# roahmlab/koopman-realizations

Hardware: AMD Instinct MI355X
Metric: EDMD snapshot-pairs/sec (bilinear fit, 3-link arm, poly-3) (higher is better)
Workload: dtype f64

## Files before the change

### koopman-realizations_amd/csrc/kp_context.hip

```cpp
#include <algorithm>
#include <cmath>
#include <cstring>
#include <mutex>

#include "kp_internal.h"

static std::mutex g_err_mu;
static std::string g_err;

void kp_set_global_error(const std::string& s) {
  std::lock_guard<std::mutex> l(g_err_mu);
  g_err = s;
}

void* kp_ctx::workspace(int slot, size_t bytes) {
  if (ws_bytes[slot] >= bytes && ws[slot]) return ws[slot];
  if (ws[slot]) (void)hipFree(ws[slot]);
  ws[slot] = nullptr;
  ws_bytes[slot] = 0;
  size_t want = bytes + bytes / 4 + 256;
  if (hipMalloc(&ws[slot], want) != hipSuccess) return nullptr;
  ws_bytes[slot] = want;
  return ws[slot];
}
// ... 94 lines not shown
  copy = g_err;
  return copy.c_str();
}

extern "C" int kp_device_info(const kp_ctx* c, char* name, int name_len, int* num_cu, int64_t* hbm) {
  if (!c) return KP_ERR_ARG;
  if (name && name_len > 0) {
    std::strncpy(name, c->name.c_str(), (size_t)name_len - 1);
    name[name_len - 1] = 0;
  }
  if (num_cu) *num_cu = c->num_cu;
  if (hbm) *hbm = c->hbm_bytes;
  return KP_OK;
}

void* kp_pinned_scratch(kp_ctx* ctx, size_t bytes) {
  if (ctx->pin_scratch_bytes >= bytes) return ctx->pin_scratch;
  if (ctx->pin_scratch) {
    (void)hipStreamSynchronize(ctx->stream);
    (void)hipHostFree(ctx->pin_scratch);
  }
  ctx->pin_scratch = nullptr;
  ctx->pin_scratch_bytes = 0;
  const size_t cap = (bytes + 4095) & ~(size_t)4095;
  if (hipHostMalloc(&ctx->pin_scratch, cap, hipHostMallocDefault) != hipSuccess) {
    ctx->pin_scratch = nullptr;
    return nullptr;
  }
  ctx->pin_scratch_bytes = cap;
  return ctx->pin_scratch;
}

extern "C" int kp_timer_get(const kp_ctx* c, int which, double* ms) {
  if (!c || !ms || which < 0 || which >= 20) return KP_ERR_ARG;
  *ms = c->timers[which];
  return KP_OK;
}

extern "C" void* kp_stream(const kp_ctx* c) { return c ? (void*)c->stream : nullptr; }


static int upload(kp_ctx* ctx, void** dst, const void* src, size_t bytes) {
  *dst = nullptr;
  if (bytes == 0) return KP_OK;
  KP_HIP(ctx, hipMalloc(dst, bytes));
  KP_HIP(ctx, hipMemcpy(*dst, src, bytes, hipMemcpyHostToDevice));
  return KP_OK;
}

extern "C" int kp_basis_desc_dims(const kp_basis_desc* d, int* nvars_out, int* nfull_out, int* N_out, int* W_out) {
  if (!d || d->nzeta < 1 || d->m < 0 || d->model_type < 0 || d->model_type > 2 || d->n_blocks < 0 ||
      (d->n_blocks && (!d->block_type || !d->block_count)))
    return KP_ERR_ARG;
  const int nvars = d->nzeta + (d->model_type == KP_MODEL_NONLINEAR ? d->m : 0);
  double nf = nvars + 1.0;
  for (int b = 0; b < d->n_blocks; ++b) {
    const int c = d->block_count[b];
    if (c < 0) return KP_ERR_ARG;
    switch (d->block_type[b]) {
      case KP_BLOCK_POLY: case KP_BLOCK_HERMITE: case KP_BLOCK_FOURIER_SPARSER: case KP_BLOCK_GAUSSIAN: nf += c; break;
      case KP_BLOCK_FOURIER: nf += std::pow((double)(2 * c + 1), (double)nvars) - 1.0; break;
      default: return KP_ERR_ARG;
    }
    if (nf > 1e6) return KP_ERR_ARG;
  }
  const int nfull = (int)std::llround(nf);
  const int N = d->k_pcs > 0 ? d->k_pcs + nvars + 1 : nfull;
// ... 430 lines not shown
```

### koopman-realizations_amd/csrc/kp_gram3.hip

```cpp
#include <algorithm>
#include <cstdlib>
#include <type_traits>
#include <vector>

#include "kp_internal.h"

#ifndef KP_RAW_STEP
#define KP_RAW_STEP 1
#endif
#define KT3 8
#define NF3 3
#define RS3 240
#define YOFF3 96
#define ZOFF3 192
#define WOFF3 196
#define SOFF3 208
#define NIDMAX3 144
#define PST3 10
#define POWBUF3 (PST3 * NIDMAX3)
#define PSIBUF3 (KT3 * RS3)
#define PSI03 (2 * POWBUF3)
#define LDS3_DOUBLES (PSI03 + 2 * PSIBUF3)
#define PCS03 LDS3_DOUBLES
#define PCSMAX3 32
#define LDS3_PCS_DOUBLES (2 * YOFF3 * 16)
#define GC03 LDS3_DOUBLES
#define GAUSSMAX3 32
#ifndef KP_PCS_REGS
#define KP_PCS_REGS 24
#endif
#define GNZMAX3 8
#define LDS3_GAUSS_DOUBLES (GAUSSMAX3 * GNZMAX3)

#include "kp_gram3_args.h"
#include "kp_gram3_cover.h"

__device__ double kp_gram3_ones[KT3] = {1.0, 1.0, 1.0, 1.0, 1.0, 1.0, 1.0, 1.0};

template <int NQ, int BM, bool PCS, bool EXT = false, bool PRE = false, bool TUP = false, bool P3 = false>
__global__ __launch_bounds__(256, 2) void kp_gram3_kernel(Gram3Args a) {
  constexpr int NWT = (BM + 1) * (BM + 2) / 2;
  static_assert(!P3 || (!PCS && !EXT && !PRE), "three-entry table: the in-kernel-lift monomial form");
  static_assert(!TUP || NWT % 2 == 0, "paired weights: an even number of weights (m = 3: 10 = 5 tuples, m = 2: 6 = 3 tuples)");
  auto wslot = [](int w) { return TUP ? 6 * (w & 1) + (w >> 1) : w - 1; };
  extern __shared__ __align__(16) double sm[];
  const BasisDev& b = a.b;
  const int tid = threadIdx.x;
  const int lane = tid & 63;
  const int wave = tid >> 6;
  const int per_xcd = gridDim.x / 8;
  const int logical = (int)blockIdx.x < per_xcd * 8 ? ((int)blockIdx.x % 8) * per_xcd + (int)blockIdx.x / 8 : (int)blockIdx.x;
  const int super = logical % a.nsuper;
  const int split = logical / a.nsuper;
  constexpr bool GRP = !PCS && !EXT && !PRE;
  const int fit = GRP ? __builtin_amdgcn_readfirstlane(split / a.nsplit_fit) : 0;
  const int split_local = split - fit * a.nsplit_fit;
  const double* const src_alpha = GRP ? a.grp[fit].alpha : a.alpha;
  const double* const src_beta = GRP ? a.grp[fit].beta : a.beta;
  const double* const src_u = GRP ? a.grp[fit].u : a.u;
  const int job = super * 4 + wave;
  const int nzm = b.nzeta + b.m;
  const int nrawrows = 2 * nzm;
  const int D = a.D;
  constexpr bool INL = !EXT && !PRE;
  const int RB = !INL ? D * PST3 : ((nrawrows + 1) * 62 + 4 * PST3 <= POWBUF3 ? 62 : 4 * PST3);
  const int CA = nrawrows * RB;

  const uint32_t* jd = a.desc + (size_t)job * (1 + NQ);
  const uint32_t jh = jd[0];
  const int lrow = (lane >> 4) * RS3, blk = (lane >> 2) & 3, lc = lane & 3;
  const int ao0 = PSI03 + lrow + 4 * (int)(jh & 255u) + lc;
  const int ao1 = PSI03 + lrow + 4 * (int)((jh >> 8) & 255u) + lc;
  const int qs = __builtin_amdgcn_readfirstlane((int)((jh >> 16) & 255u));
  int bo[NQ];
  int bo2[TUP ? NQ : 1];
// ... 15 lines not shown
    for (int w = 0; w < NWT; ++w) acc[q][w] = 0.0;

  auto item_setup = [&](int item, int (&fa_)[NF3], int& woff_) __attribute__((always_inline)) {
    const bool lvalid = item >= 0 && item < 2 * b.nfull;
    const int lside = (lvalid && item >= b.nfull) ? 1 : 0;
    const int lcol = lvalid ? item - lside * b.nfull : 0;
    const int lw = item - 2 * b.nfull;
    const bool lwt = lw >= 0 && lw < NWT - 1;
    const uint32_t r = lvalid ? a.recipes[lcol] : 0xffffffffu;
#pragma unroll
    for (int f = 0; f < NF3; ++f) {
      const int id = (int)((r >> (8 * f)) & 255u);
      fa_[f] = id == 255 ? CA : (EXT && id >= 128) ? CA + (1 + lside * a.ng + (id - 128)) * PST3 : (lside * nzm + id / D) * RB + (id % D) * PST3;
    }
    if (lwt) {
      int cnt = 0;
      for (int x = 0; x <= BM; ++x)
        for (int y = x; y <= BM; ++y) {
          if (cnt == lw + 1) {
            if (x > 0) fa_[0] = (b.nzeta + x - 1) * RB;
            if (y > 0) fa_[1] = (b.nzeta + y - 1) * RB;
          }
          ++cnt;
        }
    }
    woff_ = PSI03 + (lvalid ? lside * YOFF3 + lcol : lwt ? WOFF3 + wslot(lw + 1) : SOFF3 + (tid & 31));
  };
  constexpr int NLS = 3;
  int fs[NLS][NF3], ws[NLS];
  {
    const int nitems = 2 * b.nfull + NWT - 1;
#pragma unroll
    for (int j = 0; j < NLS; ++j) {
      const int e = tid + 256 * j;
      const bool on = e < 4 * nitems;
      const int ch = on ? e / nitems : 0;
      item_setup(on ? e - ch * nitems : -1, fs[j], ws[j]);
#pragma unroll
      for (int f = 0; f < NF3; ++f) fs[j][f] += 2 * ch;
      ws[j] += 2 * ch * RS3;
    }
  }

  const int64_t kt0 = (int64_t)split_local * a.ktiles_per_split;
  const int64_t ktiles_total = (a.Ns + KT3 - 1) / KT3;
  const int nkt = (int)max((int64_t)0, min((int64_t)a.ktiles_per_split, ktiles_total - kt0));

  constexpr int LR = 1;
  const int nld = (nrawrows * KT3 + 255) / 256;
  constexpr int LG = EXT ? 2 : 0;
  struct RawRegs { double v[LR]; bool ok; };
  bool ld_on[LR];
  bool ld_isz[LR];
  const double* ld_ptr[LR];
  const int ld_s = tid & (KT3 - 1);
  const int ld_dst0 = (tid / KT3) * RB + ld_s;
  int ld_rem = (int)max((int64_t)-1000000, min((int64_t)1 << 30, a.Ns - (kt0 * KT3 + ld_s)));
#pragma unroll
  for (int j = 0; j < LR; ++j) {
    const int e = tid + j * 256;
    ld_on[j] = e < nrawrows * KT3;
    const int r = ld_on[j] ? e / KT3 : 0;
    const int rr = r % nzm;
    const double* src = rr < b.nzeta ? ((r < nzm ? src_alpha : src_beta) + (int64_t)rr * a.Ns) : (src_u + (int64_t)(rr - b.nzeta) * a.Ns);
    ld_ptr[j] = src + kt0 * KT3 + ld_s;
    ld_isz[j] = ld_on[j] && rr < b.nzeta;
  }
  bool g_on[LG > 0 ? LG : 1];
  const double* g_ptr[LG > 0 ? LG : 1];
  int g_dst[LG > 0 ? LG : 1], g_cen[LG > 0 ? LG : 1];
  if (EXT) {
#pragma unroll
    for (int q = 0; q < LG; ++q) {
      const int gi = tid + q * 256;
      g_on[q] = gi < 2 * a.ng * KT3;
      const int gc = g_on[q] ? (gi / KT3) % a.ng : 0, gside = g_on[q] ? gi / (KT3 * a.ng) : 0;
// ... 123 lines not shown
  int pre_dst[2] = {0, 0};
  if (PRE) {
#pragma unroll
    for (int j = 0; j < 2; ++j) {
      const int e = tid + j * 256;
      pre_on[j] = e < pre_n2;
      const int e1 = pre_on[j] ? e : 0;
      const int sp = e1 / a.pre_rl, c = e1 - sp * a.pre_rl, srow = 2 * sp;
      const int cw = c - 8 * a.G4;
      const int off = c < 4 * a.G4 ? c : c < 8 * a.G4 ? YOFF3 + (c - 4 * a.G4) : WOFF3 + (!TUP ? cw : cw < NWT - 1 ? wslot(cw + 1) : (cw - (NWT - 1)) < 2 * (6 - NWT / 2) ? ((cw - (NWT - 1)) / (6 - NWT / 2)) * 6 + NWT / 2 + (cw - (NWT - 1)) % (6 - NWT / 2) : 12);
      pre_dst[j] = PSI03 + srow * RS3 + off;
    }
  }
  auto load_pre = [&]() __attribute__((always_inline)) -> PreRegs {
    PreRegs x;
    x.v[0] = make_double2(0.0, 0.0);
    x.v[1] = make_double2(0.0, 0.0);
    if (pre_left > 0) {
      if (pre_on[0]) x.v[0] = pre_ptr[0];
      if (pre_on[1]) x.v[1] = pre_ptr[256];
      pre_ptr += pre_n2;
    }
    --pre_left;
    return x;
  };
  auto store_pre = [&](auto buf_c, const PreRegs& x) __attribute__((always_inline)) {
    constexpr int BUF = decltype(buf_c)::value;
    if (pre_on[0]) { sm[BUF * PSIBUF3 + pre_dst[0]] = x.v[0].x; sm[BUF * PSIBUF3 + pre_dst[0] + RS3] = x.v[0].y; }
    if (pre_on[1]) { sm[BUF * PSIBUF3 + pre_dst[1]] = x.v[1].x; sm[BUF * PSIBUF3 + pre_dst[1] + RS3] = x.v[1].y; }
  };

  constexpr int NCH = NLS;
  double2 lf[NF3];
  auto lift_read = [&](int j, auto buf_c) __attribute__((always_inline)) {
    constexpr int BUF = decltype(buf_c)::value;
#pragma unroll
    for (int f = 0; f < NF3; ++f)
      lf[f] = *reinterpret_cast<const double2*>(__builtin_assume_aligned(&sm[BUF * POWBUF3 + fs[j][f]], 16));
  };
  auto lift_write = [&](int j, auto buf_c) __attribute__((always_inline)) {
    constexpr int BUF = decltype(buf_c)::value;
    sm[BUF * PSIBUF3 + ws[j]] = (lf[0].x * lf[1].x) * lf[2].x;
    sm[BUF * PSIBUF3 + ws[j] + RS3] = (lf[0].y * lf[1].y) * lf[2].y;
  };
  constexpr int WAIT_LGKM0 = 0xc07f;
  static_assert(WAIT_LGKM0 == ((63 & 15) | (7 << 4) | (0 << 8) | ((63 >> 4) << 14)), "vmcnt = 63 and expcnt = 7 (no wait), lgkmcnt = 0");
  auto lds_store_barrier = [&]() __attribute__((always_inline)) {
    __builtin_amdgcn_s_waitcnt(WAIT_LGKM0);
    __syncthreads();
  };
  using B0 = std::integral_constant<int, 0>;
  using B1 = std::integral_constant<int, 1>;

  constexpr int PREG = PCS ? KP_PCS_REGS : 1;
  double pcs_r[PREG];
  if (PCS) {
    __syncthreads();
    const int bbase0 = PCS03 + (lane >> 4) * 16 + 4 * blk + lc;
#pragma unroll
    for (int kk = 0; kk < PREG; ++kk) pcs_r[kk] = kk < a.nfull4 / 4 ? sm[bbase0 + kk * 64] : 0.0;
  }
  auto project = [&](auto buf_c) __attribute__((always_inline)) {
    constexpr int BUF = decltype(buf_c)::value;
    const int side = wave >> 1, rg = wave & 1;
    const int abase = BUF * PSIBUF3 + PSI03 + (4 * rg + lc) * RS3 + side * YOFF3 + (lane >> 4);
    const int bbase = PCS03 + (lane >> 4) * 16 + 4 * blk + lc;
    const int nf4 = a.nfull4;
    double p0 = 0.0, p1 = 0.0;
    const int bb1 = bbase + nf4 * 16;
    const int nk = nf4 / 4;
#pragma unroll
    for (int kk = 0; kk < PREG; ++kk) {
      if (kk < nk) {
        const double av = sm[abase + 4 * kk];
        const double b1 = sm[bb1 + kk * 64];
        p0 = __builtin_amdgcn_mfma_f64_4x4x4f64(av, pcs_r[kk], p0, 0, 0, 0);
// ... 15 lines not shown
      const int pc = 4 * blk + lc;
      if (pc < b.k_pcs) sm[srow + b.nzeta + pc] = p0;
      if (pc + 16 < b.k_pcs) sm[srow + b.nzeta + pc + 16] = p1;
    }
    if (tid < 2 * KT3) {
      sm[crow + b.N - 1] = one;
      for (int c = b.N; c < 4 * a.G4; ++c) sm[crow + c] = 0.0;
    }
    __syncthreads();
  };

  __syncthreads();
  if constexpr (PRE) {
    store_pre(B0{}, load_pre());
    __syncthreads();
  } else {
    if constexpr (INL) store_tb_v(B0{}, tb_v0, 0);
    else store_raw(B0{}, load_raw());
    lds_store_barrier();
#pragma unroll
    for (int i = 0; i < NCH; ++i) {
      lift_read(i, B0{});
      lift_write(i, B0{});
    }
    if constexpr (INL) store_tb_v(B1{}, tb_v1, 1);
    else store_raw(B1{}, load_raw());
    lds_store_barrier();
    if (PCS) project(B0{});
  }

  constexpr int NSTEP = (KT3 / 4) * NQ;
  constexpr int SP = NSTEP / NCH > 0 ? NSTEP / NCH : 1;
  constexpr int LAG = SP / 2 > 0 ? SP / 2 : 1;
  constexpr int PF_AHEAD = 3;
  constexpr int PF = NSTEP < PF_AHEAD ? NSTEP : PF_AHEAD;

  auto tile = [&](auto cur_c, auto qs_c) __attribute__((always_inline)) {
    constexpr int CUR = decltype(cur_c)::value;
    constexpr int QS = decltype(qs_c)::value;
    using NXT = std::integral_constant<int, 1 - CUR>;
    constexpr int PB = CUR * PSIBUF3;
    RawRegs rawreg;
    PreRegs prereg;
    constexpr int NAW = TUP ? NWT / 2 : NWT;
    double bvs[NSTEP];
    double bvs2[TUP ? NSTEP : 1];
    double aw[NAW];
    double wt[NAW];
    double av1 = 0.0;
    double avn0, avn1 = 0.0;
    auto weigh = [&](double av) __attribute__((always_inline)) {
#pragma unroll
      for (int w = 0; w < NAW; ++w) {
        aw[w] = (!TUP && w == 0) ? av : av * wt[w];
      }
    };
#pragma unroll
    for (int i = 0; i < PF; ++i) {
      bvs[i] = sm[PB + (i / NQ) * 4 * RS3 + bo[i % NQ]];
      if constexpr (TUP) bvs2[i] = sm[PB + (i / NQ) * 4 * RS3 + bo2[i % NQ]];
    }
    avn0 = sm[PB + ao0];
    if (QS < NQ) avn1 = sm[PB + ao1];
    auto load_wt = [&](int kk) __attribute__((always_inline)) {
      if constexpr (TUP) {
#pragma unroll
        for (int w = 0; w + 1 < NAW; w += 2) {
          const double2 v = *reinterpret_cast<const double2*>(&sm[PB + kk * 4 * RS3 + wo + w]);
          wt[w] = v.x;
          wt[w + 1] = v.y;
        }
        wt[NAW - 1] = sm[PB + kk * 4 * RS3 + wo + NAW - 1];
      } else {
#pragma unroll
        for (int w = 0; w < NWT - 1; w += 2) {
          const double2 v = *reinterpret_cast<const double2*>(&sm[PB + kk * 4 * RS3 + wo + w]);
// ... 135 lines not shown
    for (uint32_t k = dst_off[e]; k < dst_off[e + 1]; ++k) {
      const uint32_t d = dst[k];
      const size_t di = d & 0xffffu, dj = d >> 16;
      const size_t r1 = (size_t)wa * N + di, c1 = (size_t)wb * N + dj;
      const size_t r2 = (size_t)wb * N + di, c2 = (size_t)wa * N + dj;
      G[c1 * W + r1] = s; G[r1 * W + c1] = s;
      G[c2 * W + r2] = s; G[r2 * W + c2] = s;
    }
  } else if (gb < G4) {
    const int jb = 4 * gb + (l & 3);
    if (jb >= N) return;
    if (ga == gb && ia > jb) return;
    const size_t r1 = (size_t)wa * N + ia, c1 = (size_t)wb * N + jb;
    const size_t r2 = (size_t)wb * N + ia, c2 = (size_t)wa * N + jb;
    G[c1 * W + r1] = s; G[r1 * W + c1] = s;
    G[c2 * W + r2] = s; G[r2 * W + c2] = s;
  } else {
    const int jb = 4 * (gb - G4) + (l & 3);
    if (jb >= N) return;
    C[((size_t)wb * N + jb) * W + (size_t)wa * N + ia] = s;
    C[((size_t)wa * N + jb) * W + (size_t)wb * N + ia] = s;
  }
}

struct kp_gram3_plan {
  int G4 = 0, nq = 0, njobs = 0, nsuper = 0;
  int wpw = 4;
  int two_group_jobs = 0;
  uint32_t* desc = nullptr;
  uint32_t* dst_off = nullptr;
  uint32_t* dst = nullptr;
  kp_gram3_plan* cover = nullptr;
  bool cover_tried = false;
};

void kp_gram3_plan_free(kp_gram3_plan* p) {
  if (!p) return;
  kp_gram3_plan_free(p->cover);
  if (p->desc) (void)hipFree(p->desc);
  if (p->dst_off) (void)hipFree(p->dst_off);
  if (p->dst) (void)hipFree(p->dst);
  delete p;
}

static hipError_t plan3_upload(uint32_t** dev, const std::vector<uint32_t>& host) {
  hipError_t e = hipMalloc((void**)dev, std::max<size_t>(host.size(), 1) * 4);
  if (e == hipSuccess && !host.empty()) e = hipMemcpy(*dev, host.data(), host.size() * 4, hipMemcpyHostToDevice);
  return e;
}

static int make_plan3(kp_ctx* ctx, int N, int nwt, int nq_cap, kp_gram3_plan** out, int wpw = 4, int nq_force = 0) {
  kp_gram3_plan* p = new kp_gram3_plan();
  p->wpw = wpw;
  const int G4 = (N + 3) / 4;
  p->G4 = G4;
  size_t maxq = 0;
  const std::vector<std::vector<int>> rows = gram3_circulant_rows(G4, &maxq);
  Gram3JobsHost jobs;
  gram3_pack_rows(rows, G4, nwt, nq_cap, maxq, wpw, nq_force, &jobs);
  p->nq = jobs.nq;
  p->njobs = jobs.njobs;
  p->nsuper = jobs.njobs / wpw;
  p->two_group_jobs = gram3_two_group_jobs(jobs);
  hipError_t e = plan3_upload(&p->desc, jobs.desc);
  if (e != hipSuccess) {
    kp_gram3_plan_free(p);
    return ctx->fail(KP_ERR_HIP, std::string("kp_fit_gram: plan upload: ") + hipGetErrorString(e));
  }
  *out = p;
  return KP_OK;
}

static bool gram3_tup(int bm) {
  static const bool off = getenv("KP_GRAM3_NOTUP") != nullptr;
  return bm >= 2 && !off;
}

template <int NQ, int BM, bool PCS, bool EXT = false, bool PRE = false, bool TUP = false, bool P3 = false>
static hipError_t launch3c(const Gram3Args& a, int grid, size_t lds, hipStream_t st) {
  static KpLdsCache lds_cache;
  {
    const size_t lds_max = (size_t)(LDS3_DOUBLES + (PCS ? LDS3_PCS_DOUBLES : 0) + (EXT ? LDS3_GAUSS_DOUBLES : 0)) * sizeof(double);
    hipError_t e = kp_ensure_lds(lds_cache, (const void*)kp_gram3_kernel<NQ, BM, PCS, EXT, PRE, TUP, P3>, lds_max);
    if (e != hipSuccess) return e;
  }
  hipLaunchKernelGGL((kp_gram3_kernel<NQ, BM, PCS, EXT, PRE, TUP, P3>), dim3(grid), dim3(256), lds, st, a);
  return hipGetLastError();
}

template <int NQ, int BM, bool PCS, bool EXT = false, bool PRE = false>
static hipError_t launch3b(const Gram3Args& a, int grid, size_t lds, hipStream_t st) {
  if constexpr (!PCS && !EXT && !PRE) {
    if (a.pow3) return launch3c<NQ, BM, false, false, false, (BM >= 2), true>(a, grid, lds, st);
  }
  if constexpr (BM >= 2) {
    if (gram3_tup(BM)) return launch3c<NQ, BM, PCS, EXT, PRE, true>(a, grid, lds, st);
  }
  return launch3c<NQ, BM, PCS, EXT, PRE, false>(a, grid, lds, st);
}

template <int NQ>
static hipError_t launch3(const Gram3Args& a, int bm, int grid, size_t lds, hipStream_t st) {
  if (a.pre) {
    switch (bm) {
      case 1: return launch3b<NQ, 1, false, false, true>(a, grid, lds, st);
      case 2: return launch3b<NQ, 2, false, false, true>(a, grid, lds, st);
      default: return launch3b<NQ, 3, false, false, true>(a, grid, lds, st);
    }
  }
  if (a.pcs) {
    if constexpr (NQ <= 4) {
      switch (bm) {
        case 1: return launch3b<NQ, 1, true>(a, grid, lds, st);
        case 2: return launch3b<NQ, 2, true>(a, grid, lds, st);
        default: return launch3b<NQ, 3, true>(a, grid, lds, st);
      }
    } else {
      return hipErrorInvalidValue;
    }
  }
  if (a.df > 0 || a.ng > 0) {
    switch (bm) {
      case 1: return launch3b<NQ, 1, false, true>(a, grid, lds, st);
      case 2: return launch3b<NQ, 2, false, true>(a, grid, lds, st);
      default: return launch3b<NQ, 3, false, true>(a, grid, lds, st);
// ... 67 lines not shown
    const BasisDev& b = basis->dev;
    const int N = b.N, NWT = (b.m + 1) * (b.m + 2) / 2;
    if (circ.wpw != 4 || b.k_pcs != 0 || gram3_ext(basis) || !basis->fast || b.nfull != N || (int)basis->h_recipes.size() != N) return KP_OK;
    Gram3CoverHost cov;
    if (!gram3_cover_build(basis->h_recipes.data(), N, basis->pow_depth, NWT, 6, circ.wpw, &cov) || cov.jobs.njobs >= circ.njobs) return KP_OK;
    if (gram3_onea_on()) {
      Gram3CoverHost one;
      if (gram3_onea_build(basis->h_recipes.data(), N, basis->pow_depth, cov, &one) && one.jobs.nq == cov.jobs.nq && one.jobs.njobs <= cov.jobs.njobs) cov = std::move(one);
    }
    kp_gram3_plan* p = new kp_gram3_plan();
    p->G4 = circ.G4;
    p->two_group_jobs = gram3_two_group_jobs(cov.jobs);
    p->nq = cov.jobs.nq;
    p->njobs = cov.jobs.njobs;
    p->nsuper = cov.jobs.njobs / circ.wpw;
    p->cover_tried = true;
    hipError_t e = plan3_upload(&p->desc, cov.jobs.desc);
    if (e == hipSuccess) e = plan3_upload(&p->dst_off, cov.dst_off);
    if (e == hipSuccess) e = plan3_upload(&p->dst, cov.dst);
    if (e != hipSuccess) {
      kp_gram3_plan_free(p);
      circ.cover_tried = false;
      return ctx->fail(KP_ERR_HIP, std::string("kp_fit_gram: plan upload: ") + hipGetErrorString(e));
    }
    circ.cover = p;
  }
  *out = circ.cover;
  return KP_OK;
}

static bool gram3_pow3_on() {
  static const bool on = [] { const char* e = getenv("KP_GRAM3_POW3"); return !e || atoi(e) != 0; }();
  return on;
}

static int gram3_plan_for(kp_ctx* ctx, kp_basis* basis, bool deferred, kp_gram3_plan** out) {
  int rc = gram3_plan(ctx, basis);
  if (rc) return rc;
  *out = basis->plan3;
  if (gram3_cover_mode() == 2 || (gram3_cover_mode() == 1 && deferred)) {
    kp_gram3_plan* cov = nullptr;
    rc = gram3_cover_plan(ctx, basis, &cov);
    if (rc) return rc;
    if (cov) *out = cov;
  }
  return KP_OK;
}

static int64_t gram3_slots(const kp_ctx* ctx, const kp_gram3_plan& plan, int* ncu_out = nullptr, int* wgpcu_out = nullptr) {
  int ncu = ctx->num_cu > 0 ? ctx->num_cu : 256;
  int wg_per_cu = plan.wpw == 8 ? 1 : 2;
  if (const char* ov = getenv("KP_GRAM3_WGPCU")) wg_per_cu = std::max(1, atoi(ov));
  if (ncu_out) *ncu_out = ncu;
  if (wgpcu_out) *wgpcu_out = wg_per_cu;
  return (int64_t)std::max(8, ncu) * wg_per_cu;
}

bool kp_gram3_groupable(kp_ctx* ctx, const kp_basis* basis_c, const kp_snapshots* s) {
  kp_basis* basis = const_cast<kp_basis*>(basis_c);
  const BasisDev& b = basis->dev;
  if (!(kp_gram3_applicable(basis) && b.k_pcs == 0 && !gram3_ext(basis) && !gram6_on() && s->nzeta == b.nzeta && s->m == b.m)) return false;
  kp_gram3_plan* plan = nullptr;
  if (gram3_plan_for(ctx, basis, true, &plan) != KP_OK || plan->wpw == 8) return false;
  static const int64_t max_kps = [] { const char* e = getenv("KP_GRAM_GROUP_MAX_KPS"); return e ? (int64_t)atoll(e) : (int64_t)512; }();
  const int64_t ktiles = (s->Ns + KT3 - 1) / KT3, nsplit = std::max<int64_t>(1, gram3_slots(ctx, *plan) / plan->nsuper);
  return (ktiles + nsplit - 1) / nsplit < max_kps;
// ... 54 lines not shown
    }
  }
  if (pre && !ext && !basis->d_pcsT) {
    if (hipMalloc(&basis->d_pcsT, (size_t)b.nfull * 32 * 8) != hipSuccess) return ctx->fail(KP_ERR_HIP, "kp_fit_gram: out of device memory");
    KP_HIP(ctx, kp_gram3_pcs_transpose_launch(b.pcs, b.nfull, b.k_pcs, (double*)basis->d_pcsT, ctx->stream));
  }
  const size_t lds = (size_t)(LDS3_DOUBLES + (b.k_pcs > 0 && !pre ? 2 * nfull4 * 16 : 0) + (ext && !pre ? LDS3_GAUSS_DOUBLES : 0)) * sizeof(double);

  Gram3Args a;
  a.b = b;
  a.alpha = s->alpha;
  a.beta = s->beta;
  a.u = s->u;
  a.Ns = s->Ns;
  a.G4 = plan.G4;
  a.nsuper = plan.nsuper;
  a.ktiles_per_split = kps;
  a.D = ext ? basis->ext_Dp + 2 * basis->ext_df : basis->pow_depth;
  a.recipes = (const uint32_t*)(ext ? basis->d_recipes_ext : basis->d_recipes);
  a.Dp = ext ? basis->ext_Dp : basis->pow_depth;
  a.df = ext ? basis->ext_df : 0;
  a.ng = ext ? basis->ext_ng : 0;
  a.centres = b.centres;
  a.desc = plan.desc;
  a.part = part;
  a.njobs = plan.njobs;
  a.pcs = b.k_pcs > 0 && !pre ? b.pcs : nullptr;
  a.nfull4 = nfull4;
  a.pre = pre_buf;
  a.pre_rl = pre_rl;
  a.nsplit_fit = nsplit;
  for (int f = 0; f < n; ++f) a.grp[f] = Gram3Src{ss[f]->alpha, ss[f]->beta, ss[f]->u};
  a.pow3 = !pre && b.k_pcs == 0 && !ext && plan.wpw == 4 && basis->pow_depth <= 3 && (BM < 2 || gram3_tup(BM)) && gram3_pow3_on();
  const int grid = plan.nsuper * nsplit * n;
  if (!ctx->ring_timing) KP_HIP(ctx, hipEventRecord(ctx->ev0, ctx->stream));
  hipEvent_t ev_start = ctx->evp[0], ev_end = ctx->evp[1];
  const bool timed = !ctx->ring_timing || (ctx->ring_group && n > 1) || (ctx->ring_skip++ & 3) == 0;
  hipEvent_t ev_red = nullptr;
  if (ctx->ring_timing && timed) {
    ev_start = ctx->ring[2 * ctx->ring_pos];
    ev_end = ctx->ring[2 * ctx->ring_pos + 1];
    ctx->ring_members[ctx->ring_pos] = n;
    ctx->ring_has_red[ctx->ring_pos] = false;
    if (ctx->ring_group && n > 1) {
      ev_red = ctx->ring_red[ctx->ring_pos];
      ctx->ring_has_red[ctx->ring_pos] = ev_red != nullptr;
    }
    ctx->ring_pos = (ctx->ring_pos + 1) % 64;
    if (ctx->ring_n < 64) ++ctx->ring_n;
  }
  if (timed) KP_HIP(ctx, hipEventRecord(ev_start, ctx->stream));
  hipError_t e;
  if (pre && ext)
    KP_HIP(ctx, kp_gram3_prelift_ext_launch(BM, s->alpha, s->beta, s->u, s->Ns, ktiles * KT3, b.nzeta, basis->ext_Dp, basis->ext_df, basis->ext_ng, b.nfull, plan.G4,
                                            (const uint32_t*)basis->d_recipes_ext, b.centres, pre_buf, pre_rl, ctx->stream));
  else if (pre)
    KP_HIP(ctx, kp_gram3_prelift_launch(BM, s->alpha, s->beta, s->u, s->Ns, ktiles * KT3, b.nzeta, basis->pow_depth, b.nfull, b.k_pcs, N, plan.G4,
                                        (const uint32_t*)basis->d_recipes, (const double*)basis->d_pcsT, pre_buf, pre_rl, ctx->stream));
  if (plan.wpw == 8) e = kp_gram6_launch_kernel(a, plan.nq, grid, ctx->stream);
  else switch (plan.nq) {
    case 1: e = launch3<1>(a, BM, grid, lds, ctx->stream); break;
    case 2: e = launch3<2>(a, BM, grid, lds, ctx->stream); break;
    case 3: e = launch3<3>(a, BM, grid, lds, ctx->stream); break;
    case 4: e = launch3<4>(a, BM, grid, lds, ctx->stream); break;
    case 5: e = launch3<5>(a, BM, grid, lds, ctx->stream); break;
    default: e = launch3<6>(a, BM, grid, lds, ctx->stream); break;
  }
  KP_HIP(ctx, e);
  if (timed) KP_HIP(ctx, hipEventRecord(ev_end, ctx->stream));
  hipLaunchKernelGGL(kp_gram3_reduce_kernel, dim3(plan.njobs * plan.nq * NWT, n), dim3(nsplit >= 128 ? 1024 : nsplit >= 32 ? 512 : 256), 0, ctx->stream, part, nsplit, plan.njobs,
                     plan.nq, NWT, BM, plan.desc, plan.G4, N, W, GC_dev, GC_dev + (size_t)W * W, plan.wpw != 8 && gram3_tup(BM) ? 1 : 0, plan.dst_off, plan.dst);
  KP_HIP(ctx, hipGetLastError());
  if (ev_red) KP_HIP(ctx, hipEventRecord(ev_red, ctx->stream));
  if (!ctx->ring_timing) {
    KP_HIP(ctx, hipEventRecord(ctx->ev1, ctx->stream));
    KP_HIP(ctx, hipEventRecord(ctx->evp[2], ctx->stream));
  }
  ctx->gram_flops_per_pair = (double)W * (W + 1) + 2.0 * W * W;
  ctx->timers[10] = (double)plan.njobs * plan.nq * NWT * 128.0 + (b.k_pcs > 0 && !pre ? (double)plan.nsuper * nfull4 * 128.0 : 0.0);
  ctx->timers[16] = (pre || ext || plan.wpw == 8) ? 0.0 : a.pow3 ? 3.0 : 4.0;
  ctx->timers[15] = (double)plan.two_group_jobs;
  return KP_OK;
}

int kp_gram3_launch(kp_ctx* ctx, const kp_basis* basis, const kp_snapshots* s, double* GC_dev, bool cover) { return gram3_launch_n(ctx, basis, &s, 1, GC_dev, cover); }

int kp_gram3_launch_group(kp_ctx* ctx, const kp_basis* basis, const kp_snapshots* const* ss, int n, double* GC_dev) {
  return gram3_launch_n(ctx, basis, ss, n, GC_dev, true);
}


__global__ __launch_bounds__(256) void kp_gram3_linear_gather_kernel(const double* __restrict__ GCb, int N, int m, int Wb, double* __restrict__ GC) {
  const int W = N + m;
  const int e = blockIdx.x * 256 + threadIdx.x;
  if (e >= 2 * W * W) return;
  const int which = e / (W * W), r = e - which * W * W, i = r % W, j = r / W;
  const int bi = i < N ? i : (i - N + 1) * N + N - 1, bj = j < N ? j : (j - N + 1) * N + N - 1;
  GC[e] = GCb[(size_t)which * Wb * Wb + (size_t)bj * Wb + bi];
}

static kp_basis* gram3_shadow(const kp_basis* basis_c) {
  kp_basis* basis = const_cast<kp_basis*>(basis_c);
  if (!basis->shadow_bil) {
    kp_basis* sh = new kp_basis(*basis);
    sh->dev.model_type = KP_MODEL_BILINEAR;
    sh->dev.W = sh->dev.N * (sh->dev.m + 1);
    sh->plan = nullptr; sh->plan2 = nullptr; sh->plan3 = nullptr; sh->plan5 = nullptr; sh->shadow_bil = nullptr;
    sh->d_pcsT = nullptr;
    basis->shadow_bil = sh;
  }
  return basis->shadow_bil;
}

// ... 127 lines not shown
```

### koopman-realizations_amd/csrc/kp_gram3_args.h

```cpp
#pragma once
#include "kp_internal.h"

struct Gram3Src { const double *alpha, *beta, *u; };

struct Gram3Args {
  BasisDev b;
  const double* alpha;
  const double* beta;
  const double* u;
  int64_t Ns;
  int G4;
  int nsuper;
  int ktiles_per_split;
  int D;
  const uint32_t* recipes;
  const uint32_t* desc;
  double* part;
  int njobs;
  const double* pcs;
  int nfull4;
  int Dp, df, ng;
  const double* centres;
  const double* pre = nullptr;
  int pre_rl = 0;
  int nsplit_fit = 1 << 30;
  Gram3Src grp[KP_GRAM_GROUP_MAX] = {};
  bool pow3 = false;
};

bool kp_gram6_serves(int nq, int G4);
hipError_t kp_gram6_launch_kernel(const Gram3Args& a, int nq, int grid, hipStream_t st);

hipError_t kp_gram3_pcs_transpose_launch(const double* pcs, int nfull, int k, double* pcsT, hipStream_t st);
hipError_t kp_gram3_prelift_launch(int BM, const double* alpha, const double* beta, const double* u, int64_t Ns, int64_t Ns_pad, int nzeta, int D, int nfull, int k_pcs,
                                   int N, int G4, const uint32_t* recipes, const double* pcsT, double* out, int rl, hipStream_t st);
hipError_t kp_gram3_prelift_ext_launch(int BM, const double* alpha, const double* beta, const double* u, int64_t Ns, int64_t Ns_pad, int nzeta, int Dp, int df, int ng,
                                       int nfull, int G4, const uint32_t* recipes, const double* centres, double* out, int rl, hipStream_t st);
```

### koopman-realizations_amd/csrc/kp_internal.h

```cpp
#pragma once
#include <hip/hip_runtime.h>
#include <stdint.h>
#include <atomic>
#include <mutex>
#include <string>
#include <utility>
#include <vector>

#include "koopman_hip.h"

#define KP_MAX_VARS 32
#define KP_GRAM_GROUP_MAX 8

void kp_set_global_error(const std::string& s);
void kp_traj_device_blocks(kp_traj* t, double** blocks);
struct kp_comm_state;

struct kp_stage;

struct kp_ctx {
  int device = 0;
  kp_stage* stage = nullptr;
  std::vector<void*> host_blocks;
  std::vector<std::pair<void*, size_t>> traj_pool;
// ... 8 lines not shown
  int async_count = 0;
  bool batch_closed = true;
  bool kres_is_ring = false;
  const void* pend_basis = nullptr;
  int64_t pend_Ns = 0;
  int pend_W = 0;
  int pend_solves = 0, pend_first = 0;
  hipEvent_t ev_solve0 = nullptr, ev_solve1 = nullptr;
  int* sticky_info = nullptr;
  const kp_snapshots* pend_grams[KP_GRAM_GROUP_MAX] = {};
  int pend_ngrams = 0;
  const kp_basis* pend_gram_basis = nullptr;
  double* pend_gram_gc = nullptr;
  bool ring_timing = false;
  bool ring_group = false;
  unsigned ring_skip = 0;
  hipEvent_t ring[2 * 64] = {};
  int ring_pos = 0, ring_n = 0;
  hipEvent_t ring_red[64] = {};
  int ring_members[64] = {};
  bool ring_has_red[64] = {};
  kp_comm_state* comm = nullptr;
  std::atomic<bool> comm_abandoned{false};
  bool gc_preloaded = false;
  bool reduce_grams = false;
  bool test_hooks = false;
  void* pin_scratch = nullptr;
  size_t pin_scratch_bytes = 0;
  double* pin_small = nullptr;
  int num_cu = 0;
  int64_t hbm_bytes = 0;
  std::string name;
  mutable std::string err;
  double timers[20] = {0};
  double gram_flops_per_pair = 0;
  void* ws[21] = {nullptr};
  size_t ws_bytes[21] = {0};
  int last_rank = -1;
  double last_pivot_ratio = 1.0;
  double* Kres = nullptr;
  size_t Kres_bytes = 0;
  int Kres_W = 0, Kres_n = 0;
  double* GC = nullptr;
  size_t GC_bytes = 0;
  int GC_W = 0;

  int fail(int code, const std::string& s) const {
    err = s;
    kp_set_global_error(s);
    return code;
  }
  void* workspace(int slot, size_t bytes);
};

#define KP_HIP(ctx, expr)                                                                  \
  do {                                                                                     \
    hipError_t _e = (expr);                                                                \
    if (_e != hipSuccess)                                                                  \
      return (ctx)->fail(KP_ERR_HIP, std::string(#expr) + ": " + hipGetErrorString(_e));   \
  } while (0)

enum : int { COL_VAR = 0, COL_MONO = 1, COL_FOURIER = 2, COL_GAUSS = 3, COL_CONST = 4, COL_HERMITE = 5, COL_FSPARSE = 6 };

struct ColDesc {
  int32_t kind;
  int32_t arg;
  int32_t aux;
// ... 229 lines not shown
```

Measured before the change: 333.2 million.

## Reorder in-kernel lift slots so heavy three-factor monomials run first

Adds a host-built lift table that sorts lift items so every three-factor product lands in the first 256-thread step and later steps read only two factors. Factor positions are compacted per item and LDS addresses are precomputed as 32-bit address-space-3 pointers, kept in registers through asm barriers. The prefetch depth drops from 3 to 2 on this path. The aim is fewer LDS reads and multiplies per tile, paid for with extra table upload logic, higher register pressure from the pinned addresses, and the assumption that there are at most 256 heavy items.

```diff
diff --git a/koopman-realizations_amd/csrc/kp_context.hip b/koopman-realizations_amd/csrc/kp_context.hip
--- a/koopman-realizations_amd/csrc/kp_context.hip
+++ b/koopman-realizations_amd/csrc/kp_context.hip
@@ -150,7 +150,7 @@
 }
 
 extern "C" int kp_timer_get(const kp_ctx* c, int which, double* ms) {
-  if (!c || !ms || which < 0 || which >= 20) return KP_ERR_ARG;
+  if (!c || !ms || which < 0 || which >= 21) return KP_ERR_ARG;
   *ms = c->timers[which];
   return KP_OK;
 }
diff --git a/koopman-realizations_amd/csrc/kp_gram3.hip b/koopman-realizations_amd/csrc/kp_gram3.hip
--- a/koopman-realizations_amd/csrc/kp_gram3.hip
+++ b/koopman-realizations_amd/csrc/kp_gram3.hip
@@ -34,13 +34,15 @@
 
 #include "kp_gram3_args.h"
 #include "kp_gram3_cover.h"
+#include "kp_gram3_lift.h"
 
 __device__ double kp_gram3_ones[KT3] = {1.0, 1.0, 1.0, 1.0, 1.0, 1.0, 1.0, 1.0};
 
-template <int NQ, int BM, bool PCS, bool EXT = false, bool PRE = false, bool TUP = false, bool P3 = false>
+template <int NQ, int BM, bool PCS, bool EXT = false, bool PRE = false, bool TUP = false, bool P3 = false, bool LO = false>
 __global__ __launch_bounds__(256, 2) void kp_gram3_kernel(Gram3Args a) {
   constexpr int NWT = (BM + 1) * (BM + 2) / 2;
   static_assert(!P3 || (!PCS && !EXT && !PRE), "three-entry table: the in-kernel-lift monomial form");
+  static_assert(!LO || (!PCS && !EXT && !PRE), "ordered lift slots: the in-kernel-lift monomial form");
   static_assert(!TUP || NWT % 2 == 0, "paired weights: an even number of weights (m = 3: 10 = 5 tuples, m = 2: 6 = 3 tuples)");
   auto wslot = [](int w) { return TUP ? 6 * (w & 1) + (w >> 1) : w - 1; };
   extern __shared__ __align__(16) double sm[];
@@ -122,16 +124,37 @@
     const int nitems = 2 * b.nfull + NWT - 1;
 #pragma unroll
     for (int j = 0; j < NLS; ++j) {
-      const int e = tid + 256 * j;
-      const bool on = e < 4 * nitems;
-      const int ch = on ? e / nitems : 0;
-      item_setup(on ? e - ch * nitems : -1, fs[j], ws[j]);
-#pragma unroll
-      for (int f = 0; f < NF3; ++f) fs[j][f] += 2 * ch;
-      ws[j] += 2 * ch * RS3;
-    }
-  }
-
+      if constexpr (LO) {
+        const uint32_t sw = a.lift[tid + 256 * j];
+        const bool on = sw != GRAM3_LIFT_IDLE;
+        const int ch = on ? (int)((sw >> 8) & 3u) : 0;
+        int fr[NF3];
+        item_setup(on ? (int)(sw & 255u) : -1, fr, ws[j]);
+#pragma unroll
+        for (int f = 0; f < NF3; ++f) {
+          const int p = on ? (int)((sw >> (10 + 2 * f)) & 3u) : 3;
+          fs[j][f] = (p == 0 ? fr[0] : p == 1 ? fr[1] : p == 2 ? fr[2] : CA) + 2 * ch;
+        }
+        ws[j] += 2 * ch * RS3;
+      } else {
+        const int e = tid + 256 * j;
+        const bool on = e < 4 * nitems;
+        const int ch = on ? e / nitems : 0;
+        item_setup(on ? e - ch * nitems : -1, fs[j], ws[j]);
+#pragma unroll
+        for (int f = 0; f < NF3; ++f) fs[j][f] += 2 * ch;
+        ws[j] += 2 * ch * RS3;
+      }
+    }
+  }
+
+  uint32_t fsb[NLS][NF3], wsb[NLS];
+#pragma unroll
+  for (int j = 0; j < NLS; ++j) {
+#pragma unroll
+    for (int f = 0; f < NF3; ++f) fsb[j][f] = (uint32_t)(uintptr_t)(__attribute__((address_space(3))) double*)(sm + fs[j][f]);
+    wsb[j] = (uint32_t)(uintptr_t)(__attribute__((address_space(3))) double*)(sm + ws[j]);
+  }
   const int64_t kt0 = (int64_t)split_local * a.ktiles_per_split;
   const int64_t ktiles_total = (a.Ns + KT3 - 1) / KT3;
   const int nkt = (int)max((int64_t)0, min((int64_t)a.ktiles_per_split, ktiles_total - kt0));
@@ -321,16 +344,34 @@
 
   constexpr int NCH = NLS;
   double2 lf[NF3];
+  typedef double lds_d2 __attribute__((ext_vector_type(2)));
+  auto lift_nf = [](int j) { return LO && j > 0 ? 2 : NF3; };
   auto lift_read = [&](int j, auto buf_c) __attribute__((always_inline)) {
     constexpr int BUF = decltype(buf_c)::value;
 #pragma unroll
     for (int f = 0; f < NF3; ++f)
-      lf[f] = *reinterpret_cast<const double2*>(__builtin_assume_aligned(&sm[BUF * POWBUF3 + fs[j][f]], 16));
+      if (f < lift_nf(j)) {
+        if constexpr (LO) {
+          const lds_d2 v = *(const __attribute__((address_space(3))) lds_d2*)(uintptr_t)(fsb[j][f] + (uint32_t)(BUF * POWBUF3 * 8));
+          lf[f].x = v.x;
+          lf[f].y = v.y;
+        } else lf[f] = *reinterpret_cast<const double2*>(__builtin_assume_aligned(&sm[BUF * POWBUF3 + fs[j][f]], 16));
+      }
   };
   auto lift_write = [&](int j, auto buf_c) __attribute__((always_inline)) {
     constexpr int BUF = decltype(buf_c)::value;
-    sm[BUF * PSIBUF3 + ws[j]] = (lf[0].x * lf[1].x) * lf[2].x;
-    sm[BUF * PSIBUF3 + ws[j] + RS3] = (lf[0].y * lf[1].y) * lf[2].y;
+    if constexpr (LO) {
+      const double px = lift_nf(j) == 2 ? lf[0].x * lf[1].x : (lf[0].x * lf[1].x) * lf[2].x;
+      const double py = lift_nf(j) == 2 ? lf[0].y * lf[1].y : (lf[0].y * lf[1].y) * lf[2].y;
+      *(__attribute__((address_space(3))) double*)(uintptr_t)(wsb[j] + (uint32_t)(BUF * PSIBUF3 * 8)) = px;
+      *(__attribute__((address_space(3))) double*)(uintptr_t)(wsb[j] + (uint32_t)((BUF * PSIBUF3 + RS3) * 8)) = py;
+    } else if (lift_nf(j) == 2) {
+      sm[BUF * PSIBUF3 + ws[j]] = lf[0].x * lf[1].x;
+      sm[BUF * PSIBUF3 + ws[j] + RS3] = lf[0].y * lf[1].y;
+    } else {
+      sm[BUF * PSIBUF3 + ws[j]] = (lf[0].x * lf[1].x) * lf[2].x;
+      sm[BUF * PSIBUF3 + ws[j] + RS3] = (lf[0].y * lf[1].y) * lf[2].y;
+    }
   };
   constexpr int WAIT_LGKM0 = 0xc07f;
   static_assert(WAIT_LGKM0 == ((63 & 15) | (7 << 4) | (0 << 8) | ((63 >> 4) << 14)), "vmcnt = 63 and expcnt = 7 (no wait), lgkmcnt = 0");
@@ -412,7 +453,7 @@
   constexpr int NSTEP = (KT3 / 4) * NQ;
   constexpr int SP = NSTEP / NCH > 0 ? NSTEP / NCH : 1;
   constexpr int LAG = SP / 2 > 0 ? SP / 2 : 1;
-  constexpr int PF_AHEAD = 3;
+  constexpr int PF_AHEAD = LO ? 2 : 3;
   constexpr int PF = NSTEP < PF_AHEAD ? NSTEP : PF_AHEAD;
 
   auto tile = [&](auto cur_c, auto qs_c) __attribute__((always_inline)) {
@@ -422,6 +463,15 @@
     constexpr int PB = CUR * PSIBUF3;
     RawRegs rawreg;
     PreRegs prereg;
+    if constexpr (LO) {
+#pragma unroll
+      for (int j = 0; j < NLS; ++j) {
+#pragma unroll
+        for (int f = 0; f < NF3; ++f)
+          if (f < lift_nf(j)) asm volatile("" : "+v"(fsb[j][f]));
+        asm volatile("" : "+v"(wsb[j]));
+      }
+    }
     constexpr int NAW = TUP ? NWT / 2 : NWT;
     double bvs[NSTEP];
     double bvs2[TUP ? NSTEP : 1];
@@ -623,6 +673,8 @@
   uint32_t* dst = nullptr;
   kp_gram3_plan* cover = nullptr;
   bool cover_tried = false;
+  uint32_t* lift = nullptr;
+  bool lift_tried = false;
 };
 
 void kp_gram3_plan_free(kp_gram3_plan* p) {
@@ -631,6 +683,7 @@
   if (p->desc) (void)hipFree(p->desc);
   if (p->dst_off) (void)hipFree(p->dst_off);
   if (p->dst) (void)hipFree(p->dst);
+  if (p->lift) (void)hipFree(p->lift);
   delete p;
 }
 
@@ -667,21 +720,23 @@
   return bm >= 2 && !off;
 }
 
-template <int NQ, int BM, bool PCS, bool EXT = false, bool PRE = false, bool TUP = false, bool P3 = false>
+template <int NQ, int BM, bool PCS, bool EXT = false, bool PRE = false, bool TUP = false, bool P3 = false, bool LO = false>
 static hipError_t launch3c(const Gram3Args& a, int grid, size_t lds, hipStream_t st) {
   static KpLdsCache lds_cache;
   {
     const size_t lds_max = (size_t)(LDS3_DOUBLES + (PCS ? LDS3_PCS_DOUBLES : 0) + (EXT ? LDS3_GAUSS_DOUBLES : 0)) * sizeof(double);
-    hipError_t e = kp_ensure_lds(lds_cache, (const void*)kp_gram3_kernel<NQ, BM, PCS, EXT, PRE, TUP, P3>, lds_max);
+    hipError_t e = kp_ensure_lds(lds_cache, (const void*)kp_gram3_kernel<NQ, BM, PCS, EXT, PRE, TUP, P3, LO>, lds_max);
     if (e != hipSuccess) return e;
   }
-  hipLaunchKernelGGL((kp_gram3_kernel<NQ, BM, PCS, EXT, PRE, TUP, P3>), dim3(grid), dim3(256), lds, st, a);
+  hipLaunchKernelGGL((kp_gram3_kernel<NQ, BM, PCS, EXT, PRE, TUP, P3, LO>), dim3(grid), dim3(256), lds, st, a);
   return hipGetLastError();
 }
 
 template <int NQ, int BM, bool PCS, bool EXT = false, bool PRE = false>
 static hipError_t launch3b(const Gram3Args& a, int grid, size_t lds, hipStream_t st) {
   if constexpr (!PCS && !EXT && !PRE) {
+    if (a.lift) return a.pow3 ? launch3c<NQ, BM, false, false, false, (BM >= 2), true, true>(a, grid, lds, st)
+                              : launch3c<NQ, BM, false, false, false, (BM >= 2), false, true>(a, grid, lds, st);
     if (a.pow3) return launch3c<NQ, BM, false, false, false, (BM >= 2), true>(a, grid, lds, st);
   }
   if constexpr (BM >= 2) {
@@ -815,6 +870,31 @@
 static bool gram3_pow3_on() {
   static const bool on = [] { const char* e = getenv("KP_GRAM3_POW3"); return !e || atoi(e) != 0; }();
   return on;
+}
+
+static bool gram3_lift_order_on() {
+  static const bool on = [] { const char* e = getenv("KP_GRAM3_LIFT_ORDER"); return !e || atoi(e) != 0; }();
+  return on;
+}
+
+static int gram3_lift_table(kp_ctx* ctx, kp_basis* basis, const uint32_t** out) {
+  kp_gram3_plan& circ = *basis->plan3;
+  *out = nullptr;
+  if (!circ.lift_tried) {
+    const BasisDev& b = basis->dev;
+    Gram3LiftOrderHost lo;
+    if (basis->fast && (int)basis->h_recipes.size() == b.nfull && gram3_lift_order_build(basis->h_recipes.data(), b.nfull, b.m, &lo)) {
+      hipError_t e = plan3_upload(&circ.lift, lo.slot);
+      if (e != hipSuccess) {
+        if (circ.lift) (void)hipFree(circ.lift);
+        circ.lift = nullptr;
+        return ctx->fail(KP_ERR_HIP, std::string("kp_fit_gram: lift table upload: ") + hipGetErrorString(e));
+      }
+    }
+    circ.lift_tried = true;
+  }
+  *out = circ.lift;
+  return KP_OK;
 }
 
 static int gram3_plan_for(kp_ctx* ctx, kp_basis* basis, bool deferred, kp_gram3_plan** out) {
@@ -935,6 +1015,10 @@
   a.nsplit_fit = nsplit;
   for (int f = 0; f < n; ++f) a.grp[f] = Gram3Src{ss[f]->alpha, ss[f]->beta, ss[f]->u};
   a.pow3 = !pre && b.k_pcs == 0 && !ext && plan.wpw == 4 && basis->pow_depth <= 3 && (BM < 2 || gram3_tup(BM)) && gram3_pow3_on();
+  if (!pre && b.k_pcs == 0 && !ext && plan.wpw == 4 && (BM < 2 || gram3_tup(BM)) && gram3_lift_order_on()) {
+    int rc = gram3_lift_table(ctx, basis, &a.lift);
+    if (rc) return rc;
+  }
   const int grid = plan.nsuper * nsplit * n;
   if (!ctx->ring_timing) KP_HIP(ctx, hipEventRecord(ctx->ev0, ctx->stream));
   hipEvent_t ev_start = ctx->evp[0], ev_end = ctx->evp[1];
@@ -982,6 +1066,7 @@
   ctx->gram_flops_per_pair = (double)W * (W + 1) + 2.0 * W * W;
   ctx->timers[10] = (double)plan.njobs * plan.nq * NWT * 128.0 + (b.k_pcs > 0 && !pre ? (double)plan.nsuper * nfull4 * 128.0 : 0.0);
   ctx->timers[16] = (pre || ext || plan.wpw == 8) ? 0.0 : a.pow3 ? 3.0 : 4.0;
+  ctx->timers[20] = a.lift ? 1.0 : 0.0;
   ctx->timers[15] = (double)plan.two_group_jobs;
   return KP_OK;
 }
diff --git a/koopman-realizations_amd/csrc/kp_gram3_args.h b/koopman-realizations_amd/csrc/kp_gram3_args.h
--- a/koopman-realizations_amd/csrc/kp_gram3_args.h
+++ b/koopman-realizations_amd/csrc/kp_gram3_args.h
@@ -26,6 +26,7 @@
   int nsplit_fit = 1 << 30;
   Gram3Src grp[KP_GRAM_GROUP_MAX] = {};
   bool pow3 = false;
+  const uint32_t* lift = nullptr;
 };
 
 bool kp_gram6_serves(int nq, int G4);
diff --git a/koopman-realizations_amd/csrc/kp_gram3_lift.h b/koopman-realizations_amd/csrc/kp_gram3_lift.h
--- /dev/null
+++ b/koopman-realizations_amd/csrc/kp_gram3_lift.h
@@ -0,0 +1,69 @@
+#pragma once
+#include <cstdint>
+#include <vector>
+
+#define GRAM3_LIFT_STEPS 3
+#define GRAM3_LIFT_SLOTS (GRAM3_LIFT_STEPS * 256)
+#define GRAM3_LIFT_IDLE 0xffffffffu
+
+static inline uint32_t gram3_lift_word(int item, int pair, const int p[3], int nreal) {
+  return (uint32_t)item | (uint32_t)pair << 8 | (uint32_t)p[0] << 10 | (uint32_t)p[1] << 12 | (uint32_t)p[2] << 14 | (uint32_t)nreal << 16;
+}
+
+static inline void gram3_lift_factors(const uint32_t* recipes, int nfull, int bm, int item, bool real[3]) {
+  if (item < 2 * nfull) {
+    const uint32_t r = recipes[item < nfull ? item : item - nfull];
+    for (int f = 0; f < 3; ++f) real[f] = ((r >> (8 * f)) & 255u) != 255u;
+    return;
+  }
+  const int lw = item - 2 * nfull;
+  int cnt = 0;
+  real[0] = real[1] = real[2] = false;
+  for (int x = 0; x <= bm; ++x)
+    for (int y = x; y <= bm; ++y) {
+      if (cnt == lw + 1) {
+        real[0] = x > 0;
+        real[1] = y > 0;
+      }
+      ++cnt;
+    }
+}
+
+struct Gram3LiftOrderHost {
+  bool ordered = false;
+  int njobs = 0, heavy = 0, two = 0, light = 0;
+  std::vector<uint32_t> slot;
+};
+
+static inline bool gram3_lift_order_build(const uint32_t* recipes, int nfull, int bm, Gram3LiftOrderHost* out) {
+  *out = Gram3LiftOrderHost();
+  if (nfull < 1 || bm < 1 || bm > 3) return false;
+  const int nwt = (bm + 1) * (bm + 2) / 2, nitems = 2 * nfull + nwt - 1;
+  out->njobs = 4 * nitems;
+  if (out->njobs > GRAM3_LIFT_SLOTS) return false;
+  for (int c = 0; c < nfull; ++c)
+    if ((recipes[c] >> 24) != 255u) return false;
+  std::vector<uint32_t> heavy, rest;
+  for (int e = 0; e < out->njobs; ++e) {
+    const int pair = e / nitems, item = e - pair * nitems;
+    bool real[3];
+    gram3_lift_factors(recipes, nfull, bm, item, real);
+    int p[3] = {3, 3, 3}, n = 0;
+    for (int f = 0; f < 3; ++f)
+      if (real[f]) p[n++] = f;
+    const uint32_t w = gram3_lift_word(item, pair, p, n);
+    if (n == 3) {
+      heavy.push_back(w);
+      ++out->heavy;
+    } else {
+      rest.push_back(w);
+      ++(n == 2 ? out->two : out->light);
+    }
+  }
+  if (heavy.size() > 256) return false;
+  out->slot = heavy;
+  out->slot.insert(out->slot.end(), rest.begin(), rest.end());
+  out->slot.resize(GRAM3_LIFT_SLOTS, GRAM3_LIFT_IDLE);
+  out->ordered = true;
+  return true;
+}
diff --git a/koopman-realizations_amd/csrc/kp_internal.h b/koopman-realizations_amd/csrc/kp_internal.h
--- a/koopman-realizations_amd/csrc/kp_internal.h
+++ b/koopman-realizations_amd/csrc/kp_internal.h
@@ -64,7 +64,7 @@
   int64_t hbm_bytes = 0;
   std::string name;
   mutable std::string err;
-  double timers[20] = {0};
+  double timers[21] = {0};
   double gram_flops_per_pair = 0;
   void* ws[21] = {nullptr};
   size_t ws_bytes[21] = {0};
```

New measurement: 336.6 million, median of 6. 1.0% higher.
